# Liz490/multimodal_alzheimer

Hardware: AMD Instinct MI355X
Metric: volumes/sec fwd+bwd, 3D-ResNet-10 @128^3 bf16, 1/2/4/8 MI355X; % HBM roofline (higher is better)
Workload: dtype bf16; 1 GPU; BASELINE config 2: Anat_CNN ResNet-10 MRI-only, 1x128^3, batch 8/GPU, weighted CE, Adam, fwd+bwd+step; global_batch=8, parallelism=dp1, step_launch=hip graph replay

## Files before the change

### multimodal_alzheimer_amd/csrc/patchz.hip

```cpp
#include <atomic>
#include <cstdlib>
#include <type_traits>
#include <utility>

#include "common.h"
#include "patchconv.h"

namespace {

constexpr int PX = 10, PY = 10;
constexpr int RB = 128;
constexpr int PROWS = PX * PY;
constexpr int PSLOT = 104 * RB;
constexpr int NPS = 8;
constexpr int WSLOT = 64 * RB;
constexpr int NST = 4;
constexpr int RING_OFF = NPS * PSLOT;
constexpr int STG_OFF = RING_OFF + NST * WSLOT;
constexpr int CROW = 64 * 2 + 16;
constexpr int STG_BYTES = 128 * CROW;
constexpr int RED_OFF = STG_OFF + STG_BYTES;
constexpr int LDS = RED_OFF + (8 - 1) * 128 * 4;
static_assert(LDS <= 160 * 1024, "LDS budget");
constexpr int NTHR = 512, NW = 8;
constexpr int TAPS = 27;

struct PZ {
  int nb, Nd, Kpad, D, H, W;
  int nty, ntx, nbn, nseg, tps;
  const u16* res;
  int relu;
};

__device__ const u32x4 g_zero16z[8] = {};
constexpr int EPI_ST = 4;
constexpr int STATS_ST = 8;

__device__ __forceinline__ void st_u32x4(void* p, u32x4 v) {
  asm volatile("global_store_dwordx4 %0, %1, off\n\ts_nop 1" ::"v"(p), "v"(v) : "memory");
}
__device__ __forceinline__ void st_f32(float* p, float v) {
  asm volatile("global_store_dword %0, %1, off\n\ts_nop 1" ::"v"(p), "v"(v) : "memory");
}
__device__ __forceinline__ void lds_barrier() {
  asm volatile("s_waitcnt lgkmcnt(0)" ::: "memory");
  __builtin_amdgcn_s_barrier();
  asm volatile("" ::: "memory");
}

__host__ __device__ constexpr int planes_at(int r) { return r == 0 ? 2 : (r == 9 || r == 18) ? 1 : 0; }
template <int T, bool NEXT, bool PREV_NEXT, bool LAST>
__host__ __device__ constexpr int younger() {
  int n = 0;
  for (int d = 1; d <= 2; ++d) {
    const int r = T - d;
    const bool next = r >= 0 ? NEXT : PREV_NEXT;
    const int rr = r >= 0 ? r : r + TAPS;
    n += 2 * (next ? planes_at(rr) : 0);
    const bool w = !(LAST && r + 4 >= TAPS);
    n += w ? 1 : 0;
  }
  return n;
}

__global__ __launch_bounds__(NTHR) void patchz_conv_kernel(PZ g, const u16* __restrict__ src,
                                                           const u16* __restrict__ wgt,
                                                           const float* __restrict__ bias,
                                                           u16* __restrict__ dst,
                                                           float* __restrict__ stats) {
  extern __shared__ __attribute__((aligned(16))) char smem[];
  const int tid = threadIdx.x, lane = tid & 63;
  const int wave = __builtin_amdgcn_readfirstlane(tid >> 6);
  const int nwg = gridDim.x, bid = blockIdx.x;
  const int xcd = bid & 7, qq = nwg >> 3, rr = nwg & 7;
  const int item = (xcd < rr ? xcd * (qq + 1) : rr * (qq + 1) + (xcd - rr) * qq) + (bid >> 3);
  int t1 = item;
  const int seg = t1 % g.nseg;
  t1 /= g.nseg;
  const int nt = t1 % g.nbn;
  t1 /= g.nbn;
  const int bx = t1 % g.ntx;
  t1 /= g.ntx;
  const int by = t1 % g.nty;
  const int n = t1 / g.nty;
  const int y0 = by * 8, x0 = bx * 8, n0 = nt * 64;
  const int zs = seg * g.tps * 4;
  const int HW = g.H * g.W;

  const u16* __restrict__ srcn = src + (int64_t)n * g.D * HW * 64;
  int poff[2];
  uint32_t pdst[2];
  {
    const int lrow = lane >> 3;
#pragma unroll
    for (int h = 0; h < 2; ++h) {
      const int p = min(wave + NW * h, 12);
      const int r = p * 8 + lrow;
      const int px = r % PX, py = r / PX;
      const int y = y0 - 1 + py, x = x0 - 1 + px;
      const bool in = r < PROWS && (unsigned)y < (unsigned)g.H && (unsigned)x < (unsigned)g.W;
      const int chunk = (lane & 7) ^ (px & 7);
      poff[h] = in ? (y * g.W + x) * 64 + chunk * 8 : -1;
      pdst[h] = p * 1024;
    }
  }
  auto issue_plane = [&](int q) __attribute__((always_inline)) {
    const int z = zs - 1 + q;
    const bool zin = (unsigned)z < (unsigned)g.D;
    const u16* base = srcn + (int64_t)(zin ? z : 0) * HW * 64;
    char* slot = smem + (q & (NPS - 1)) * PSLOT;
#pragma unroll
    for (int h = 0; h < 2; ++h) {
      const void* p = (zin && poff[h] >= 0) ? (const void*)(base + poff[h]) : (const void*)g_zero16z;
      glds16_asm(p, lds_addr_of(slot + pdst[h]));
    }
  };
  const int lrow = lane >> 3;
  const u16* wrow = wgt + (int64_t)(n0 + wave * 8 + lrow) * g.Kpad + (((lane & 7) ^ lrow) * 8);
  auto issue_w = [&](int gt, int wt) __attribute__((always_inline)) {
    glds16_asm(wrow + wt * 64,
               lds_addr_of(smem + RING_OFF + (gt & (NST - 1)) * WSLOT + wave * 1024));
  };

  const int wz = wave >> 1;
  const int lr = lane & 15, lk = lane >> 4;
  const int tx = lr & 7, ty0 = 4 * (wave & 1) + (lr >> 3);
  uint32_t aoff[3][2];
#pragma unroll
  for (int kx = 0; kx < 3; ++kx)
#pragma unroll
    for (int k = 0; k < 2; ++k)
      aoff[kx][k] = (uint32_t)((ty0 * PX + tx + kx) * RB + (((4 * k + lk) ^ ((tx + kx) & 7)) << 4));
  uint32_t boff[2];
#pragma unroll
  for (int k = 0; k < 2; ++k) boff[k] = (uint32_t)(lr * RB + (((4 * k + lk) ^ (lr & 7)) << 4));

  f32x4 acc[2][4];
  bf16x8 fa0[2], fb0[4], fa1[2], fb1[4];
#if defined(PZ_NO_AREAD) || defined(PZ_NO_BREAD)
#pragma unroll
  for (int i = 0; i < 2; ++i) { asm volatile("" : "=v"(fa0[i])); asm volatile("" : "=v"(fa1[i])); }
#pragma unroll
  for (int j = 0; j < 4; ++j) { asm volatile("" : "=v"(fb0[j])); asm volatile("" : "=v"(fb1[j])); }
#endif
  auto read_frags = [&](auto tc, auto kc, int q0, int gt, bf16x8 (&A)[2], bf16x8 (&B)[4])
      __attribute__((always_inline)) {
    constexpr int T = decltype(tc)::value, K = decltype(kc)::value;
    constexpr int kz = T / 9, ky = (T / 3) % 3, kx = T % 3;
    int pbase = __builtin_amdgcn_readfirstlane(((q0 + wz + kz) & (NPS - 1)) * PSLOT);
    int wbase = __builtin_amdgcn_readfirstlane(RING_OFF + (gt & (NST - 1)) * WSLOT);
    asm volatile("" : "+s"(pbase), "+s"(wbase));
    const char* pa = smem + pbase + aoff[kx][K] + ky * PX * RB;
#ifndef PZ_NO_AREAD
#pragma unroll
    for (int i = 0; i < 2; ++i)
      A[i] = *reinterpret_cast<const bf16x8*>(pa + i * 2 * PX * RB);
#endif
    const char* pb = smem + wbase + boff[K];
#ifndef PZ_NO_BREAD
#pragma unroll
    for (int j = 0; j < 4; ++j) B[j] = *reinterpret_cast<const bf16x8*>(pb + j * 16 * RB);
#endif
  };
  auto mma = [&](const bf16x8 (&A)[2], const bf16x8 (&B)[4]) __attribute__((always_inline)) {
#ifdef PZ_NO_MMA
#pragma unroll
    for (int i = 0; i < 2; ++i) asm volatile("" ::"v"(A[i]));
#pragma unroll
    for (int j = 0; j < 4; ++j) asm volatile("" ::"v"(B[j]));
#else
#pragma unroll
    for (int i = 0; i < 2; ++i)
#pragma unroll
      for (int j = 0; j < 4; ++j)
        acc[i][j] = __builtin_amdgcn_mfma_f32_16x16x32_bf16(A[i], B[j], acc[i][j], 0, 0, 0);
#endif
  };

  float bv[4];
#pragma unroll
  for (int j = 0; j < 4; ++j) {
    bv[j] = bias != nullptr ? bias[n0 + j * 16 + lr] : 0.f;
    asm volatile("" ::"v"(bv[j]));
  }
  const int64_t nbase = (int64_t)n * g.D;
  auto epilogue = [&](int i) __attribute__((always_inline)) {
#ifdef PZ_NO_EPI
#pragma unroll
    for (int a = 0; a < 2; ++a)
#pragma unroll
      for (int j = 0; j < 4; ++j) asm volatile("" ::"v"(acc[a][j]));
    return;
#endif
    const int z0 = zs + 4 * i;
    u16* ctile = reinterpret_cast<u16*>(smem + STG_OFF);
    float cs[4], cq[4];
#pragma unroll
    for (int j = 0; j < 4; ++j) {
      cs[j] = 0.f;
      cq[j] = 0.f;
#pragma unroll
      for (int i2 = 0; i2 < 2; ++i2)
#pragma unroll
        for (int r = 0; r < 4; ++r) {
          const float v = acc[i2][j][r] + bv[j];
          cs[j] += v;
          cq[j] += v * v;
        }
    }
    if (stats != nullptr) {
      float* red = reinterpret_cast<float*>(smem + RED_OFF);
#pragma unroll
      for (int j = 0; j < 4; ++j) {
        cs[j] += __shfl_xor(cs[j], 16, 64);
        cs[j] += __shfl_xor(cs[j], 32, 64);
        cq[j] += __shfl_xor(cq[j], 16, 64);
        cq[j] += __shfl_xor(cq[j], 32, 64);
      }
      if (wave > 0 && lk == 0) {
#pragma unroll
        for (int j = 0; j < 4; ++j) {
          red[(wave - 1) * 128 + j * 16 + lr] = cs[j];
          red[(wave - 1) * 128 + 64 + j * 16 + lr] = cq[j];
        }
      }
      lds_barrier();
      if (wave == 0) {
        const int64_t mt = (((int64_t)n * (g.D / 4) + z0 / 4) * g.nty + by) * g.ntx + bx;
        float* srow = stats + (mt * 2) * g.Nd + n0 + lr;
#pragma unroll
        for (int j = 0; j < 4; ++j) {
          float ss = cs[j], qs = cq[j];
          for (int w = 1; w < NW; ++w) {
            ss += red[(w - 1) * 128 + j * 16 + lr];
            qs += red[(w - 1) * 128 + 64 + j * 16 + lr];
          }
          st_f32(srow + j * 16, ss);
          st_f32(srow + g.Nd + j * 16, qs);
        }
      }
    }
#pragma unroll
    for (int hh = 0; hh < 2; ++hh) {
      if ((wave >> 2) == hh) {
#pragma unroll
        for (int j = 0; j < 4; ++j) {
          const int col = j * 16 + lr;
#pragma unroll
          for (int i2 = 0; i2 < 2; ++i2)
#pragma unroll
            for (int r = 0; r < 4; ++r) {
              const int row = (wave & 3) * 32 + i2 * 16 + lk * 4 + r;
              ctile[row * (CROW / 2) + col] = f2bf(acc[i2][j][r] + bv[j]);
            }
        }
      }
      lds_barrier();
#pragma unroll
      for (int h = 0; h < 2; ++h) {
        const int qd = tid + NTHR * h;
        const int row = qd >> 3, c8 = qd & 7;
        const int v = hh * 128 + row;
        const int64_t vox = ((nbase + z0 + (v >> 6)) * g.H + y0 + ((v >> 3) & 7)) * g.W + x0 + (v & 7);
        const int64_t o = vox * g.Nd + n0 + c8 * 8;
        u32x4 val = *reinterpret_cast<const u32x4*>(reinterpret_cast<const char*>(ctile) +
                                                    row * CROW + c8 * 16);
        if (g.res != nullptr || g.relu) val = epi_res_relu(val, g.res ? g.res + o : nullptr, g.relu);
        st_u32x4(dst + o, val);
      }
      lds_barrier();
    }
  };

  for (int q = 0; q < 6; ++q) issue_plane(q);
#pragma unroll
  for (int t = 0; t < NST; ++t) issue_w(t, t);
  wait_vm_lgkm0<NST - 1>();
  raw_barrier();
  read_frags(std::integral_constant<int, 0>{}, std::integral_constant<int, 0>{}, 0, 0, fa0, fb0);

  auto box = [&](int i, auto nextc, auto lastc) __attribute__((always_inline)) {
    constexpr bool NEXT = decltype(nextc)::value, LAST = decltype(lastc)::value;
    const int q0 = 4 * i, gt0 = TAPS * i;
#pragma unroll
    for (int a = 0; a < 2; ++a)
#pragma unroll
      for (int j = 0; j < 4; ++j) acc[a][j] = f32x4{0.f, 0.f, 0.f, 0.f};
    auto tap = [&](auto tc) __attribute__((always_inline)) {
      constexpr int T = decltype(tc)::value;
      const int gt = gt0 + T;
      read_frags(tc, std::integral_constant<int, 1>{}, q0, gt, fa1, fb1);
      mma(fa0, fb0);
      if constexpr (!(LAST && T == TAPS - 1)) {
        constexpr int Y = younger<T, NEXT, true, LAST>();
        if constexpr (T <= 2) {
          if (i == 0) {
            wait_vm_lgkm0<Y>();
          } else if (wave == 0 && stats != nullptr) {
            wait_vm_lgkm0<Y + EPI_ST + STATS_ST>();
          } else {
            wait_vm_lgkm0<Y + EPI_ST>();
          }
        } else {
          wait_vm_lgkm0<Y>();
        }
#ifndef PZ_NO_BAR
        raw_barrier();
#endif
        if constexpr (NEXT && planes_at(T) == 2) {
          issue_plane(q0 + 6);
          issue_plane(q0 + 7);
        } else if constexpr (NEXT && T == 9) {
          issue_plane(q0 + 8);
        } else if constexpr (NEXT && T == 18) {
          issue_plane(q0 + 9);
        }
        if constexpr (!(LAST && T + 4 >= TAPS)) issue_w(gt + 4, (T + 4) % TAPS);
        if constexpr (T + 1 < TAPS)
          read_frags(std::integral_constant<int, T + 1>{}, std::integral_constant<int, 0>{}, q0,
                     gt + 1, fa0, fb0);
        else
          read_frags(std::integral_constant<int, 0>{}, std::integral_constant<int, 0>{}, q0 + 4,
                     gt + 1, fa0, fb0);
      }
      mma(fa1, fb1);
    };
    [&]<int... T>(std::integer_sequence<int, T...>) {
      (tap(std::integral_constant<int, T>{}), ...);
    }(std::make_integer_sequence<int, TAPS>{});
    epilogue(i);
  };
  for (int i = 0; i + 1 < g.tps; ++i) box(i, std::true_type{}, std::false_type{});
  box(g.tps - 1, std::false_type{}, std::true_type{});
}

std::atomic<int> g_patchz_mode{-1};
int patchz_mode() {
  int v = g_patchz_mode.load(std::memory_order_relaxed);
  if (v < 0) {
    const char* e = getenv("MMAD_PATCHZ");
    int expect = -1;
    g_patchz_mode.compare_exchange_strong(expect, e ? atoi(e) : 1);
    v = g_patchz_mode.load(std::memory_order_relaxed);
  }
  return v;
}

int segments(const mmad_patch::Geo& q) {
  const int64_t cols = (int64_t)q.nb * (q.Hd / 8) * (q.Wd / 8) * (q.Nd / 64);
  const int boxes = q.Dd / 4;
  int s = 1;
  while (cols * s < 256 && boxes % (2 * s) == 0 && boxes / (2 * s) >= 2) s *= 2;
  return s;
}

}

namespace mmad_patchz {

int set_mode(int v) {
  const int prev = patchz_mode();
  if (v >= 0) g_patchz_mode.store(v, std::memory_order_relaxed);
  return prev;
}

bool ok(const mmad_patch::Geo& q) {
  if (patchz_mode() <= 0) return false;
  if (q.Cs != 64 || q.Nd % 64 || q.Kpad < 27 * 64) return false;
  if (q.KD != 3 || q.KH != 3 || q.KW != 3 || q.dd != 1 || q.dh != 1 || q.dw != 1) return false;
  if (q.pd != 1 || q.ph != 1 || q.pw != 1) return false;
  if (q.Ds != q.Dd || q.Hs != q.Hd || q.Ws != q.Wd) return false;
  if (q.Dd % 4 || q.Hd % 8 || q.Wd % 8) return false;
  const int s = segments(q);
  if (q.Dd / 4 / s < 2) return false;
  const int64_t cols = (int64_t)q.nb * (q.Hd / 8) * (q.Wd / 8) * (q.Nd / 64);
  if (patchz_mode() == 1 && cols * s < 256) return false;
  return (int64_t)q.Ds * q.Hs * q.Ws * 64 < (int64_t(1) << 31) &&
         (int64_t)q.nb * q.Dd * q.Hd * q.Wd * q.Nd < (int64_t(1) << 40);
}

int64_t tiles(const mmad_patch::Geo& q) {
  return (int64_t)q.nb * (q.Dd / 4) * (q.Hd / 8) * (q.Wd / 8);
}

int fwd(const mmad_patch::Geo& q, const void* src, const void* wp, const float* bias, void* dst,
        float* stats, void* stream) {
  if (!mmad_patchz::ok(q)) return MMAD_EUNSUPPORTED;
  static const bool attr =
      hipFuncSetAttribute((const void*)patchz_conv_kernel,
                          hipFuncAttributeMaxDynamicSharedMemorySize, LDS) == hipSuccess;
  if (!attr) return MMAD_EUNSUPPORTED;
  PZ g{};
  g.nb = q.nb; g.Nd = q.Nd; g.Kpad = q.Kpad; g.D = q.Dd; g.H = q.Hd; g.W = q.Wd;
  g.nty = q.Hd / 8; g.ntx = q.Wd / 8; g.nbn = q.Nd / 64;
  g.nseg = segments(q);
  g.tps = q.Dd / 4 / g.nseg;
  g.res = reinterpret_cast<const u16*>(q.res);
  g.relu = q.relu;
  const int64_t items = (int64_t)q.nb * g.nty * g.ntx * g.nbn * g.nseg;
  hipLaunchKernelGGL(patchz_conv_kernel, dim3((unsigned)items), dim3(NTHR), LDS,
                     as_stream(stream), g, (const u16*)src, (const u16*)wp, bias, (u16*)dst,
                     stats);
  return launch_status();
}

}
```

Before: 2771 volumes/sec.

## Restructure patch conv pipeline into 3-tap weight stages with deeper fragment prefetch

Reworks the implicit-GEMM 3D conv main loop. Weights now load in 3-tap stages on a 3-slot ring, and the plane ring shrinks from 8 to 6 slots with modular slot tracking. LDS fragment reads are prefetched two half-taps ahead with an explicit MFMA/DS-read interleave, and barriers happen once per stage instead of once per tap. The BN-stats reduction is also moved so two waves finish it after the staging barrier, which drops a barrier and shares LDS with the staging buffer. This trades more VGPRs and trickier slot bookkeeping for fewer syncs and better latency hiding.

```diff
diff --git a/multimodal_alzheimer_amd/csrc/patchz.hip b/multimodal_alzheimer_amd/csrc/patchz.hip
--- a/multimodal_alzheimer_amd/csrc/patchz.hip
+++ b/multimodal_alzheimer_amd/csrc/patchz.hip
@@ -12,18 +12,24 @@
 constexpr int RB = 128;
 constexpr int PROWS = PX * PY;
 constexpr int PSLOT = 104 * RB;
-constexpr int NPS = 8;
+constexpr int NPS = 6;
 constexpr int WSLOT = 64 * RB;
-constexpr int NST = 4;
+constexpr int SSLOT = 3 * WSLOT;
+constexpr int NST = 3;
 constexpr int RING_OFF = NPS * PSLOT;
-constexpr int STG_OFF = RING_OFF + NST * WSLOT;
+constexpr int STG_OFF = RING_OFF + 2 * SSLOT;
 constexpr int CROW = 64 * 2 + 16;
 constexpr int STG_BYTES = 128 * CROW;
-constexpr int RED_OFF = STG_OFF + STG_BYTES;
-constexpr int LDS = RED_OFF + (8 - 1) * 128 * 4;
+static_assert(STG_BYTES <= SSLOT, "staging aliases one weight slot");
+constexpr int RED_OFF = RING_OFF + NST * SSLOT;
+constexpr int LDS = RED_OFF + 8 * 128 * 4;
 static_assert(LDS <= 160 * 1024, "LDS budget");
 constexpr int NTHR = 512, NW = 8;
-constexpr int TAPS = 27;
+constexpr int TAPS = 27, STAGES = 9;
+constexpr int HT = 2 * TAPS;
+constexpr int PD = 2;
+constexpr int NS = PD + 1;
+static_assert(HT % NS == 0 && PD >= 1 && PD < 6, "set of a half-tap is the same in every box");
 
 struct PZ {
   int nb, Nd, Kpad, D, H, W;
@@ -34,7 +40,7 @@
 
 __device__ const u32x4 g_zero16z[8] = {};
 constexpr int EPI_ST = 4;
-constexpr int STATS_ST = 8;
+constexpr int STATS_ST = 1;
 
 __device__ __forceinline__ void st_u32x4(void* p, u32x4 v) {
   asm volatile("global_store_dwordx4 %0, %1, off\n\ts_nop 1" ::"v"(p), "v"(v) : "memory");
@@ -48,19 +54,10 @@
   asm volatile("" ::: "memory");
 }
 
-__host__ __device__ constexpr int planes_at(int r) { return r == 0 ? 2 : (r == 9 || r == 18) ? 1 : 0; }
-template <int T, bool NEXT, bool PREV_NEXT, bool LAST>
+__host__ __device__ constexpr int planes_at(int g) { return g == 8 ? 2 : (g == 2 || g == 5) ? 1 : 0; }
+template <int G, bool NEXT>
 __host__ __device__ constexpr int younger() {
-  int n = 0;
-  for (int d = 1; d <= 2; ++d) {
-    const int r = T - d;
-    const bool next = r >= 0 ? NEXT : PREV_NEXT;
-    const int rr = r >= 0 ? r : r + TAPS;
-    n += 2 * (next ? planes_at(rr) : 0);
-    const bool w = !(LAST && r + 4 >= TAPS);
-    n += w ? 1 : 0;
-  }
-  return n;
+  return G == 0 ? 2 * planes_at(STAGES - 1) : NEXT ? 2 * planes_at(G - 1) : 0;
 }
 
 __global__ __launch_bounds__(NTHR) void patchz_conv_kernel(PZ g, const u16* __restrict__ src,
@@ -104,11 +101,12 @@
       pdst[h] = p * 1024;
     }
   }
-  auto issue_plane = [&](int q) __attribute__((always_inline)) {
+  auto mod6 = [](int x) __attribute__((always_inline)) { return x >= NPS ? x - NPS : x; };
+  auto issue_plane = [&](int q, int ps) __attribute__((always_inline)) {
     const int z = zs - 1 + q;
     const bool zin = (unsigned)z < (unsigned)g.D;
     const u16* base = srcn + (int64_t)(zin ? z : 0) * HW * 64;
-    char* slot = smem + (q & (NPS - 1)) * PSLOT;
+    char* slot = smem + ps * PSLOT;
 #pragma unroll
     for (int h = 0; h < 2; ++h) {
       const void* p = (zin && poff[h] >= 0) ? (const void*)(base + poff[h]) : (const void*)g_zero16z;
@@ -117,9 +115,13 @@
   };
   const int lrow = lane >> 3;
   const u16* wrow = wgt + (int64_t)(n0 + wave * 8 + lrow) * g.Kpad + (((lane & 7) ^ lrow) * 8);
-  auto issue_w = [&](int gt, int wt) __attribute__((always_inline)) {
-    glds16_asm(wrow + wt * 64,
-               lds_addr_of(smem + RING_OFF + (gt & (NST - 1)) * WSLOT + wave * 1024));
+  auto issue_w = [&](auto gc) __attribute__((always_inline)) {
+    constexpr int G = decltype(gc)::value;
+    static_assert(G >= 0 && G < STAGES);
+#pragma unroll
+    for (int k = 0; k < 3; ++k)
+      glds16_asm(wrow + (3 * G + k) * 64,
+                 lds_addr_of(smem + RING_OFF + (G % NST) * SSLOT + k * WSLOT + wave * 1024));
   };
 
   const int wz = wave >> 1;
@@ -136,19 +138,22 @@
   for (int k = 0; k < 2; ++k) boff[k] = (uint32_t)(lr * RB + (((4 * k + lk) ^ (lr & 7)) << 4));
 
   f32x4 acc[2][4];
-  bf16x8 fa0[2], fb0[4], fa1[2], fb1[4];
+  bf16x8 fa[NS][2], fb[NS][4];
 #if defined(PZ_NO_AREAD) || defined(PZ_NO_BREAD)
 #pragma unroll
-  for (int i = 0; i < 2; ++i) { asm volatile("" : "=v"(fa0[i])); asm volatile("" : "=v"(fa1[i])); }
-#pragma unroll
-  for (int j = 0; j < 4; ++j) { asm volatile("" : "=v"(fb0[j])); asm volatile("" : "=v"(fb1[j])); }
-#endif
-  auto read_frags = [&](auto tc, auto kc, int q0, int gt, bf16x8 (&A)[2], bf16x8 (&B)[4])
+  for (int s = 0; s < NS; ++s) {
+#pragma unroll
+    for (int i = 0; i < 2; ++i) asm volatile("" : "=v"(fa[s][i]));
+#pragma unroll
+    for (int j = 0; j < 4; ++j) asm volatile("" : "=v"(fb[s][j]));
+  }
+#endif
+  auto read_frags = [&](auto tc, auto kc, int pslot, bf16x8 (&A)[2], bf16x8 (&B)[4])
       __attribute__((always_inline)) {
     constexpr int T = decltype(tc)::value, K = decltype(kc)::value;
-    constexpr int kz = T / 9, ky = (T / 3) % 3, kx = T % 3;
-    int pbase = __builtin_amdgcn_readfirstlane(((q0 + wz + kz) & (NPS - 1)) * PSLOT);
-    int wbase = __builtin_amdgcn_readfirstlane(RING_OFF + (gt & (NST - 1)) * WSLOT);
+    constexpr int ky = (T / 3) % 3, kx = T % 3;
+    int pbase = pslot;
+    int wbase = RING_OFF + ((T / 3) % NST) * SSLOT + kx * WSLOT;
     asm volatile("" : "+s"(pbase), "+s"(wbase));
     const char* pa = smem + pbase + aoff[kx][K] + ky * PX * RB;
 #ifndef PZ_NO_AREAD
@@ -208,8 +213,8 @@
           cq[j] += v * v;
         }
     }
+    float* red = reinterpret_cast<float*>(smem + RED_OFF);
     if (stats != nullptr) {
-      float* red = reinterpret_cast<float*>(smem + RED_OFF);
 #pragma unroll
       for (int j = 0; j < 4; ++j) {
         cs[j] += __shfl_xor(cs[j], 16, 64);
@@ -217,26 +222,11 @@
         cq[j] += __shfl_xor(cq[j], 16, 64);
         cq[j] += __shfl_xor(cq[j], 32, 64);
       }
-      if (wave > 0 && lk == 0) {
+      if (lk == 0) {
 #pragma unroll
         for (int j = 0; j < 4; ++j) {
-          red[(wave - 1) * 128 + j * 16 + lr] = cs[j];
-          red[(wave - 1) * 128 + 64 + j * 16 + lr] = cq[j];
-        }
-      }
-      lds_barrier();
-      if (wave == 0) {
-        const int64_t mt = (((int64_t)n * (g.D / 4) + z0 / 4) * g.nty + by) * g.ntx + bx;
-        float* srow = stats + (mt * 2) * g.Nd + n0 + lr;
-#pragma unroll
-        for (int j = 0; j < 4; ++j) {
-          float ss = cs[j], qs = cq[j];
-          for (int w = 1; w < NW; ++w) {
-            ss += red[(w - 1) * 128 + j * 16 + lr];
-            qs += red[(w - 1) * 128 + 64 + j * 16 + lr];
-          }
-          st_f32(srow + j * 16, ss);
-          st_f32(srow + g.Nd + j * 16, qs);
+          red[wave * 128 + j * 16 + lr] = cs[j];
+          red[wave * 128 + 64 + j * 16 + lr] = cq[j];
         }
       }
     }
@@ -256,6 +246,13 @@
         }
       }
       lds_barrier();
+      if (hh == 0 && stats != nullptr && wave < 2) {
+        float s = red[tid];
+#pragma unroll
+        for (int w = 1; w < NW; ++w) s += red[w * 128 + tid];
+        const int64_t mt = (((int64_t)n * (g.D / 4) + z0 / 4) * g.nty + by) * g.ntx + bx;
+        st_f32(stats + (mt * 2 + wave) * g.Nd + n0 + lane, s);
+      }
 #pragma unroll
       for (int h = 0; h < 2; ++h) {
         const int qd = tid + NTHR * h;
@@ -268,35 +265,41 @@
         if (g.res != nullptr || g.relu) val = epi_res_relu(val, g.res ? g.res + o : nullptr, g.relu);
         st_u32x4(dst + o, val);
       }
-      lds_barrier();
+      if (hh == 0) lds_barrier();
     }
   };
 
-  for (int q = 0; q < 6; ++q) issue_plane(q);
-#pragma unroll
-  for (int t = 0; t < NST; ++t) issue_w(t, t);
-  wait_vm_lgkm0<NST - 1>();
+  for (int q = 0; q < NPS; ++q) issue_plane(q, q);
+  issue_w(std::integral_constant<int, 0>{});
+  issue_w(std::integral_constant<int, 1>{});
+  wait_vm_lgkm0<3>();
   raw_barrier();
-  read_frags(std::integral_constant<int, 0>{}, std::integral_constant<int, 0>{}, 0, 0, fa0, fb0);
-
-  auto box = [&](int i, auto nextc, auto lastc) __attribute__((always_inline)) {
+  [&]<int... H>(std::integer_sequence<int, H...>) {
+    (read_frags(std::integral_constant<int, H / 2>{}, std::integral_constant<int, H % 2>{},
+                __builtin_amdgcn_readfirstlane(wz * PSLOT), fa[H], fb[H]), ...);
+  }(std::make_integer_sequence<int, PD>{});
+
+  auto box = [&](int i, int sb, auto nextc, auto lastc) __attribute__((always_inline)) {
     constexpr bool NEXT = decltype(nextc)::value, LAST = decltype(lastc)::value;
-    const int q0 = 4 * i, gt0 = TAPS * i;
+    const int q0 = 4 * i;
+    int ps[4];
+#pragma unroll
+    for (int kz = 0; kz < 3; ++kz)
+      ps[kz] = __builtin_amdgcn_readfirstlane(mod6(sb + wz + kz) * PSLOT);
+    ps[3] = __builtin_amdgcn_readfirstlane(mod6(mod6(sb + 4) + wz) * PSLOT);
 #pragma unroll
     for (int a = 0; a < 2; ++a)
 #pragma unroll
       for (int j = 0; j < 4; ++j) acc[a][j] = f32x4{0.f, 0.f, 0.f, 0.f};
-    auto tap = [&](auto tc) __attribute__((always_inline)) {
-      constexpr int T = decltype(tc)::value;
-      const int gt = gt0 + T;
-      read_frags(tc, std::integral_constant<int, 1>{}, q0, gt, fa1, fb1);
-      mma(fa0, fb0);
-      if constexpr (!(LAST && T == TAPS - 1)) {
-        constexpr int Y = younger<T, NEXT, true, LAST>();
-        if constexpr (T <= 2) {
+    auto half = [&](auto hc) __attribute__((always_inline)) {
+      constexpr int H = decltype(hc)::value;
+      constexpr int G = H / 6;
+      if constexpr (H % 6 == 6 - PD && !(LAST && G == STAGES - 1)) {
+        constexpr int Y = younger<G, NEXT>();
+        if constexpr (G == 0) {
           if (i == 0) {
-            wait_vm_lgkm0<Y>();
-          } else if (wave == 0 && stats != nullptr) {
+            wait_vm_lgkm0<0>();
+          } else if (wave < 2 && stats != nullptr) {
             wait_vm_lgkm0<Y + EPI_ST + STATS_ST>();
           } else {
             wait_vm_lgkm0<Y + EPI_ST>();
@@ -307,31 +310,45 @@
 #ifndef PZ_NO_BAR
         raw_barrier();
 #endif
-        if constexpr (NEXT && planes_at(T) == 2) {
-          issue_plane(q0 + 6);
-          issue_plane(q0 + 7);
-        } else if constexpr (NEXT && T == 9) {
-          issue_plane(q0 + 8);
-        } else if constexpr (NEXT && T == 18) {
-          issue_plane(q0 + 9);
+        if constexpr (!(LAST && G + 2 >= STAGES))
+          issue_w(std::integral_constant<int, (G + 2) % STAGES>{});
+        if constexpr (NEXT && G == 2) {
+          issue_plane(q0 + 6, sb);
+        } else if constexpr (NEXT && G == 5) {
+          issue_plane(q0 + 7, sb + 1);
+        } else if constexpr (NEXT && G == 8) {
+          issue_plane(q0 + 8, mod6(sb + 2));
+          issue_plane(q0 + 9, mod6(sb + 3));
         }
-        if constexpr (!(LAST && T + 4 >= TAPS)) issue_w(gt + 4, (T + 4) % TAPS);
-        if constexpr (T + 1 < TAPS)
-          read_frags(std::integral_constant<int, T + 1>{}, std::integral_constant<int, 0>{}, q0,
-                     gt + 1, fa0, fb0);
-        else
-          read_frags(std::integral_constant<int, 0>{}, std::integral_constant<int, 0>{}, q0 + 4,
-                     gt + 1, fa0, fb0);
-      }
-      mma(fa1, fb1);
+      } else if constexpr (H % 6 == 6 - PD && LAST && G == STAGES - 1) {
+        lds_barrier();
+      }
+      constexpr int N = H + PD;
+      if constexpr (N < HT)
+        read_frags(std::integral_constant<int, N / 2>{}, std::integral_constant<int, N % 2>{},
+                   ps[N / 18], fa[N % NS], fb[N % NS]);
+      else if constexpr (!LAST)
+        read_frags(std::integral_constant<int, (N - HT) / 2>{},
+                   std::integral_constant<int, (N - HT) % 2>{}, ps[3], fa[N % NS], fb[N % NS]);
+      mma(fa[H % NS], fb[H % NS]);
+#pragma unroll
+      for (int k = 0; k < 6; ++k) {
+        __builtin_amdgcn_sched_group_barrier(0x008, 1, 0);
+        __builtin_amdgcn_sched_group_barrier(0x100, 1, 0);
+      }
+      __builtin_amdgcn_sched_group_barrier(0x008, 2, 0);
     };
-    [&]<int... T>(std::integer_sequence<int, T...>) {
-      (tap(std::integral_constant<int, T>{}), ...);
-    }(std::make_integer_sequence<int, TAPS>{});
+    [&]<int... H>(std::integer_sequence<int, H...>) {
+      (half(std::integral_constant<int, H>{}), ...);
+    }(std::make_integer_sequence<int, HT>{});
     epilogue(i);
   };
-  for (int i = 0; i + 1 < g.tps; ++i) box(i, std::true_type{}, std::false_type{});
-  box(g.tps - 1, std::false_type{}, std::true_type{});
+  int sb = 0;
+  for (int i = 0; i + 1 < g.tps; ++i) {
+    box(i, sb, std::true_type{}, std::false_type{});
+    sb = sb >= 2 ? sb - 2 : sb + 4;
+  }
+  box(g.tps - 1, sb, std::false_type{}, std::true_type{});
 }
 
 std::atomic<int> g_patchz_mode{-1};
```

Result: faster. 2802 volumes/sec (median of 6 runs) (+1.1%).
